# wangshiwen-ai-hku/video-styler

Measured on AMD Instinct MI355X. Metric: denoising steps/sec, Wan2.1-VACE-14B 832x480x73, higher is better.
Workload: dtype bf16; 1 GPU; Wan2.1-VACE-14B 832x480x73: 40 DiT + 8 VACE blocks, CFG 5.0 as one batch-2 forward + Euler; model=Wan2.1-VACE-14B, global_batch=1, seq_len=29640, parallelism=single, lora=merged (zero runtime cost, as the reference's GeneralLoRALoader), step_exec=hipGraph replay, sampler=flow-match Euler, cfg 5.0, shift 5.0

## Files before the change

video-styler_amd/csrc/attention_w4.hip:

```cpp
#include <cstdlib>
#include <mutex>
#include <set>
#include <type_traits>

#include "attention.h"

namespace vs_attn {
namespace {

constexpr int W4_THR = 256;
constexpr int W4_TILE = BKV * HD * 2;
constexpr int W4_SLOT = 2 * W4_TILE;
constexpr int W4_LDS = 4 * W4_SLOT;
constexpr int W4_QSLOT = W4_LDS;
constexpr int W4_LDS_BASE = W4_LDS + 16;
#ifdef VS_W4_STAMPS
__device__ unsigned long long g_w4_stamps[4][32][7];
constexpr int W4_SWN = 9;
__device__ unsigned long long g_w4_sw[4][16][W4_SWN];
constexpr int W4_STAMP_OFF = W4_LDS_BASE;
constexpr int W4_SW_OFF = W4_STAMP_OFF + 4 * 32 * 7 * 8;
constexpr int W4_LDS_ALLOC = W4_SW_OFF + 4 * 16 * W4_SWN * 8;
#else
constexpr int W4_LDS_ALLOC = W4_LDS_BASE;
#endif

struct AttnChunks {
    int nmain, npers;
    __device__ __forceinline__ void of(int x, int& cs, int& csz, int& gs) const {
        const int qx = nmain >> 3, rx = nmain & 7, qb = npers >> 3, rb = npers & 7;
        cs = x < rx ? x * (qx + 1) : rx * (qx + 1) + (x - rx) * qx;
        csz = qx + (x < rx ? 1 : 0);
        gs = qb + (x < rb ? 1 : 0);
    }
    __device__ __forceinline__ int take(unsigned* q, unsigned t0, int nxt, int lane) const {
        const int x = blockIdx.x & 7;
        int cs, csz, gs;
        of(x, cs, csz, gs);
        if (!q) return nxt + gs < cs + csz ? nxt + gs : -1;
        const unsigned t = vs_queue_value<0>(t0);
        if ((int)t < csz) return cs + (int)t;
        for (int it = 0; it < 16; ++it) {
            int vcs, vcsz, vgs;
            of((x + 1 + lane) & 7, vcs, vcsz, vgs);
            unsigned h = 0x7fffffff;
            if (lane < 7) h = __hip_atomic_load(q + ((x + 1 + lane) & 7) * VS_Q_LINE, __ATOMIC_RELAXED,
                                                __HIP_MEMORY_SCOPE_AGENT);
            const unsigned long long live = __ballot(lane < 7 && (int)h < vcsz);
            if (!live) return -1;
            const int v = (x + 1 + (int)__builtin_ctzll(live)) & 7;
            unsigned tv = 0;
            if (lane == 0) tv = vs_queue_add(q + v * VS_Q_LINE);
            tv = (unsigned)__builtin_amdgcn_readfirstlane((int)tv);
            of(v, vcs, vcsz, vgs);
            if ((int)tv < vcsz) return vcs + (int)tv;
        }
        return -1;
    }
};

template <bool REBASE>
__global__ __launch_bounds__(W4_THR, 1) void attn_fwd_w4(const AttnArgs args) {
    extern __shared__ __attribute__((aligned(16))) char smem[];
    typedef const volatile AttnArgs __attribute__((address_space(4))) ColdArgs;
    ColdArgs* cold = (ColdArgs*)__builtin_amdgcn_kernarg_segment_ptr();
    const int Sq = args.Sq, Skv_all = args.Skv, nmain = args.nmain, npers = args.npers;
    const int nsplit = args.nsplit, piece_tiles = args.piece_tiles;
    const long long ldq = args.ldq, ldk = args.ldk, ldv = args.ldv, ldo = args.ldo;
    const float c = args.c;

    int piece = -1, kv_begin = 0, Skv = Skv_all;
    int cur;
    const bool pers = (int)blockIdx.x < npers;
    const AttnChunks chunks{nmain, npers};
    const int tid = threadIdx.x, lane = tid & 63;
    if (pers) {
        int cs, csz, gs;
        chunks.of(blockIdx.x & 7, cs, csz, gs);
        cur = (int)(blockIdx.x >> 3) < csz ? cs + (int)(blockIdx.x >> 3) : -1;
    } else {
        const int t = blockIdx.x - npers;
        cur = nmain + t / nsplit;
        piece = t % nsplit;
        kv_begin = piece * piece_tiles * BKV;
        Skv = min(Skv_all - kv_begin, piece_tiles * BKV);
    }
    const int wave = __builtin_amdgcn_readfirstlane(tid >> 6);
    if (pers && args.queue) {
        volatile LDS_AS int* qs = (volatile LDS_AS int*)(uintptr_t)((unsigned)(uintptr_t)smem + W4_QSLOT);
        if (wave == 0) {
            const unsigned t0 = vs_queue_issue(args.queue + (blockIdx.x & 7) * VS_Q_LINE);
            const int id = chunks.take(args.queue, t0, -1, lane);
            if (lane == 0) *qs = id;
        }
        __syncthreads();
        cur = __builtin_amdgcn_readfirstlane(*qs);
    }
    if (cur < 0) {
        if (pers && args.queue && tid == 0) vs_queue_done(args.queue, 9, npers);
        return;
    }
    const int r = lane & 31, hh = lane >> 5;

    auto item_bh = [&](int g, int& qrow0) {
        const int nqb = cold->nqb;
        qrow0 = (g % nqb) * BQ;
        return g / nqb;
    };
    auto q_base = [&](int bh) { const int H = cold->H; return cold->Q + (long long)(bh / H) * cold->bsq + (bh % H) * HD; };
    auto k_base = [&](int bh) {
        const int H = cold->H;
        return cold->K + (long long)(bh / H) * cold->bsk + (long long)kv_begin * ldk + (bh % H) * HD;
    };
    auto v_base = [&](int bh) {
        const int H = cold->H;
        return cold->V + (long long)(bh / H) * cold->bsv + (long long)kv_begin * ldv + (bh % H) * HD;
    };
    auto o_base = [&](int bh) { const int H = cold->H; return cold->O + (long long)(bh / H) * cold->bso + (bh % H) * HD; };

    const int nkv = (Skv + BKV - 1) / BKV;
    const float npad = (float)(nkv * BKV - Skv);

    const int ldk32 = (int)ldk, ldv32 = (int)ldv;
    unsigned kvo[4], vvo[4];
#pragma unroll
    for (int i = 0; i < 4; ++i) {
        const int R = 16 * wave + 4 * i + (lane >> 4), p = lane & 15;
        kvo[i] = (unsigned)(R * ldk32 * 2 + ((p ^ (R & 15)) << 4));
        vvo[i] = (unsigned)(R * ldv32 * 2 + ((p ^ ((R & 3) << 2)) << 4));
    }
    auto rsrc4 = [&](const bf16_t* base, unsigned bytes) {
        const unsigned long long a = (unsigned long long)(uintptr_t)base;
        return i32x4_t{(int)(unsigned)a, (int)((unsigned)(a >> 32) & 0xffffu), (int)bytes, 0x00020000};
    };
    auto slab_rsrc = [&](const bf16_t* base, int ld) {
        return rsrc4(base, REBASE ? 0u : (unsigned)((Skv - 1) * ld * 2 + HD * 2));
    };
    auto dma16 = [](unsigned lds, unsigned voff, i32x4_t rs, int soff) __attribute__((always_inline)) {
        asm volatile("s_mov_b32 m0, %0\n\ts_nop 0\n\tbuffer_load_dwordx4 %1, %2, %3 offen lds"
                     :: "s"(lds), "v"(voff), "s"(rs), "s"(soff) : "m0");
    };
    int li = 0;
    int dnext = -1;
    int qrow_unused;
    const bf16_t* Kl = k_base(item_bh(cur, qrow_unused));
    const bf16_t* Vl = v_base(item_bh(cur, qrow_unused));
    i32x4_t krs = slab_rsrc(Kl, ldk32), vrs = slab_rsrc(Vl, ldv32);
    const unsigned lds0 = (unsigned)(uintptr_t)smem + wave * 16 * 256;
    struct StageCtx { unsigned kdst, vdst; i32x4_t kr, vr; int ks, vs; } sc;
    auto stage_begin = [&](int T) __attribute__((always_inline)) {
        sc.kdst = lds0 + (T & 3) * W4_SLOT;
        sc.vdst = sc.kdst + W4_TILE;
        const int kv0 = li * BKV;
        sc.kr = krs;
        sc.vr = vrs;
        sc.ks = kv0 * ldk32 * 2;
        sc.vs = kv0 * ldv32 * 2;
        if constexpr (REBASE) {
            const int rows = min(BKV, Skv - kv0);
            sc.kr = rsrc4(Kl + (long long)kv0 * ldk, (unsigned)((rows - 1) * ldk32 * 2 + HD * 2));
            sc.vr = rsrc4(Vl + (long long)kv0 * ldv, (unsigned)((rows - 1) * ldv32 * 2 + HD * 2));
            sc.ks = 0;
            sc.vs = 0;
        }
    };
    auto stage_piece = [&](int i) __attribute__((always_inline)) {
        if (i < 4)
            dma16(sc.kdst + i * 1024, kvo[i], sc.kr, sc.ks);
        else
            dma16(sc.vdst + (i - 4) * 1024, vvo[i - 4], sc.vr, sc.vs);
    };
    auto piece_go = [&](int i) __attribute__((always_inline)) {
        if (i < 4)
            asm volatile("buffer_load_dwordx4 %0, %1, %2 offen lds" :: "v"(kvo[i]), "s"(sc.kr), "s"(sc.ks) : "memory");
        else
            asm volatile("buffer_load_dwordx4 %0, %1, %2 offen lds" :: "v"(vvo[i - 4]), "s"(sc.vr), "s"(sc.vs) : "memory");
    };
    auto m0_step = [&](int i) __attribute__((always_inline)) {
        if (i == 4) asm volatile("s_add_u32 m0, m0, %0" :: "i"(W4_TILE - 3 * 1024) : "memory");
        else asm volatile("s_add_u32 m0, m0, 0x400" ::: "memory");
    };
    auto stage_next = [&]() __attribute__((always_inline)) {
        if (++li == nkv) {
            li = 0;
            if (dnext >= 0) {
                const int bh = item_bh(dnext, qrow_unused);
                Kl = k_base(bh);
                Vl = v_base(bh);
                krs = slab_rsrc(Kl, ldk32);
                vrs = slab_rsrc(Vl, ldv32);
                dnext = -1;
            }
        }
    };
    auto stage = [&](int T) __attribute__((always_inline)) {
        stage_begin(T);
#pragma unroll
        for (int i = 0; i < 8; ++i) stage_piece(i);
        stage_next();
    };

    bf16x8_t qf[2][8];
    auto load_q = [&](const bf16_t* qb0, int q0v) __attribute__((always_inline)) {
        bf16x8_t raw[2][8];
#pragma unroll
        for (int rb = 0; rb < 2; ++rb) {
            const int qrow = min(q0v + 32 * rb + r, Sq - 1);
            const bf16_t* src = qb0 + (long long)qrow * ldq + 8 * hh;
#pragma unroll
            for (int j = 0; j < 8; ++j) raw[rb][j] = *reinterpret_cast<const bf16x8_t*>(src + 16 * j);
        }
#pragma unroll
        for (int rb = 0; rb < 2; ++rb)
#pragma unroll
            for (int j = 0; j < 8; ++j) {
#pragma unroll
                for (int e = 0; e < 8; ++e) qf[rb][j][e] = (__bf16)((float)raw[rb][j][e] * c);
                asm volatile("" : "+a"(qf[rb][j]));
            }
    };

    int koff[8], voff[4];
#pragma unroll
    for (int j = 0; j < 8; ++j) {
        koff[j] = r * 256 + (((2 * j + hh) ^ (r & 15)) << 4);
        asm volatile("" : "+v"(koff[j]));
    }
    {
        const int g4 = lane >> 4, q4 = (lane & 15) >> 2, p4 = lane & 3;
#pragma unroll
        for (int dt = 0; dt < 4; ++dt) {
            voff[dt] = W4_TILE + (4 * (g4 >> 1) + q4) * 256 + ((dt ^ q4) << 6) + 32 * (g4 & 1) + 8 * p4;
            asm volatile("" : "+v"(voff[dt]));
        }
    }
    const unsigned smem_base = (unsigned)(uintptr_t)smem;
    auto lds16 = [&](unsigned addr) {
        return *reinterpret_cast<const LDS_AS bf16x8_t*>((const LDS_AS char*)(uintptr_t)addr);
    };
    auto tr8 = [&](unsigned addr) {
        return __builtin_amdgcn_ds_read_tr16_b64_v4i16((LDS_AS i16x4_t*)(uintptr_t)addr);
    };

    f32x16_t o[2][4];
#pragma unroll
    for (int rb = 0; rb < 2; ++rb)
#pragma unroll
        for (int dt = 0; dt < 4; ++dt)
#pragma unroll
            for (int i = 0; i < 16; ++i) o[rb][dt][i] = 0.f;
    float lsum[2] = {0.f, 0.f};
    auto row_sum = [&](int rb) { return lsum[rb] + __shfl_xor(lsum[rb], 32); };
    f32x16_t zero;
#pragma unroll
    for (int i = 0; i < 16; ++i) zero[i] = 0.f;


    auto finish = [&](bf16_t* ob, int qrow0, int gi) __attribute__((always_inline)) {
        float lt[2];
#pragma unroll
        for (int rb = 0; rb < 2; ++rb) lt[rb] = row_sum(rb) - npad;
        if (piece >= 0) {
            float* pp = args.part + ((long long)(gi - nmain) * nsplit + piece) * BQ * PROW + wave * 64 * PROW;
#pragma unroll
            for (int rb = 0; rb < 2; ++rb) {
                float* pr = pp + (32 * rb + r) * PROW;
#pragma unroll
                for (int dt = 0; dt < 4; ++dt)
#pragma unroll
                    for (int gi4 = 0; gi4 < 4; ++gi4)
                        *reinterpret_cast<f32x4_t*>(pr + 32 * dt + 8 * gi4 + 4 * hh) =
                            f32x4_t{o[rb][dt][4 * gi4], o[rb][dt][4 * gi4 + 1], o[rb][dt][4 * gi4 + 2],
                                    o[rb][dt][4 * gi4 + 3]};
                if (hh == 0) *reinterpret_cast<f32x2_t*>(pr + HD) = f32x2_t{0.f, lt[rb]};
            }
            return;
        }
        const bool ok = lt[0] >= W4_LMIN && lt[0] <= NC_LMAX && lt[1] >= W4_LMIN && lt[1] <= NC_LMAX;
        if (__any(!ok) && lane == 0) nc_list_item(cold->flags, cold->nc_cap, gi);
#pragma unroll
        for (int rb = 0; rb < 2; ++rb) {
            const float inv = 1.f / lt[rb];
            const int row = qrow0 + 32 * rb + r;
            bf16_t* op = ob + (long long)row * ldo + 8 * hh;
#pragma unroll
            for (int dt = 0; dt < 4; ++dt)
#pragma unroll
                for (int gp = 0; gp < 2; ++gp) {
                    const int gi = 2 * gp;
                    const unsigned ax = pack2(o[rb][dt][4 * gi] * inv, o[rb][dt][4 * gi + 1] * inv);
                    const unsigned ay = pack2(o[rb][dt][4 * gi + 2] * inv, o[rb][dt][4 * gi + 3] * inv);
                    const unsigned bx = pack2(o[rb][dt][4 * gi + 4] * inv, o[rb][dt][4 * gi + 5] * inv);
                    const unsigned by = pack2(o[rb][dt][4 * gi + 6] * inv, o[rb][dt][4 * gi + 7] * inv);
                    const auto sx = __builtin_amdgcn_permlane32_swap(ax, bx, false, false);
                    const auto sy = __builtin_amdgcn_permlane32_swap(ay, by, false, false);
                    if (row < Sq)
                        *reinterpret_cast<u32x4_t*>(op + 16 * (2 * dt + gp)) = u32x4_t{sx[0], sy[0], sx[1], sy[1]};
                }
        }
    };

    bf16x8_t kf0[8], kf1[8], vfa[8], vfb[8];
    f32x16_t s0[2], s1a[2], s1b[2];
    u32x4_t p0a[2][2], p0b[2][2], p1[2][2];
    auto fence = [] { __builtin_amdgcn_sched_barrier(0); };
#ifdef VS_W4_STAMPS
    unsigned long long stv[7] = {0, 0, 0, 0, 0, 0, 0};
    int st_it = -1;
    auto stamp = [&](int k) __attribute__((always_inline)) {
        if (st_it >= 0) asm volatile("s_memtime %0" : "=s"(stv[k]));
    };
    auto stamp_store = [&](int st, int lo, int hi) __attribute__((always_inline)) {
        if (st >= 0 && lane == 0)
            for (int k = lo; k < hi; ++k)
                *reinterpret_cast<volatile LDS_AS unsigned long long*>(
                    (LDS_AS char*)(uintptr_t)(smem_base + W4_STAMP_OFF + 8 * ((wave * 32 + st) * 7 + k))) = stv[k];
    };
    unsigned long long swv[W4_SWN] = {};
    int sw_i = 0;
    auto swst = [&](int k) __attribute__((always_inline)) {
        if (blockIdx.x == 0 && sw_i < 16) asm volatile("s_memtime %0\n\ts_waitcnt lgkmcnt(0)" : "=s"(swv[k]) :: "memory");
    };
    auto sw_store = [&]() __attribute__((always_inline)) {
        if (blockIdx.x == 0 && sw_i < 16) {
            asm volatile("s_waitcnt lgkmcnt(0)" ::: "memory");
            if (lane == 0)
                for (int k = 0; k < W4_SWN; ++k)
                    *reinterpret_cast<volatile LDS_AS unsigned long long*>(
                        (LDS_AS char*)(uintptr_t)(smem_base + W4_SW_OFF + 8 * ((wave * 16 + sw_i) * W4_SWN + k))) = swv[k];
        }
        ++sw_i;
    };
#else
    auto stamp = [](int) {};
    auto swst = [](int) {};
    auto sw_store = [] {};
#endif
    unsigned kbs[8], vbs[4];
    auto kbase = [&](int T) __attribute__((always_inline)) {
#pragma unroll
        for (int j = 0; j < 8; ++j) {
            kbs[j] = smem_base + (T & 3) * W4_SLOT + koff[j];
            asm volatile("" : "+v"(kbs[j]));
        }
    };
    auto vbase = [&](int T) __attribute__((always_inline)) {
#pragma unroll
        for (int dt = 0; dt < 4; ++dt) vbs[dt] = smem_base + (T & 3) * W4_SLOT + voff[dt];
    };
    auto rdK = [&](bf16x8_t& d, int kb, int j) __attribute__((always_inline)) {
        d = lds16(kbs[j] + kb * 32 * 256);
    };
    auto rdV = [&](bf16x8_t& d, int ks, int dt) __attribute__((always_inline)) {
        const unsigned a0 = vbs[dt] + ks * 16 * 256;
        const i16x4_t v0 = tr8(a0), v1 = tr8(a0 + 8 * 256);
        d = __builtin_shufflevector(__builtin_bit_cast(bf16x4_t, v0), __builtin_bit_cast(bf16x4_t, v1), 0, 1, 2,
                                    3, 4, 5, 6, 7);
    };
    auto mfV = [&](const bf16x8_t& vf, const u32x4_t (&pkv)[2][2], int ksl, int dt) __attribute__((always_inline)) {
#pragma unroll
        for (int rb = 0; rb < 2; ++rb)
        {
            o[rb][dt] = __builtin_amdgcn_mfma_f32_32x32x16_bf16(vf, __builtin_bit_cast(bf16x8_t, pkv[rb][ksl]),
                                                                 o[rb][dt], 0, 0, 0);
            asm volatile("" : "+a"(o[rb][dt]));
        }
    };
    auto mfV1 = [&](const bf16x8_t& vf, const u32x4_t (&pkv)[2][2], int ksl, int dt, int rb) __attribute__((always_inline)) {
        o[rb][dt] = __builtin_amdgcn_mfma_f32_32x32x16_bf16(vf, __builtin_bit_cast(bf16x8_t, pkv[rb][ksl]), o[rb][dt], 0, 0, 0);
        asm volatile("" : "+a"(o[rb][dt]));
    };
    auto smp = [&](const f32x16_t& sv, int e, u32x4_t (&pkd)[2], int rb) __attribute__((always_inline)) {
        const float pa = __builtin_amdgcn_exp2f(sv[e]), pb = __builtin_amdgcn_exp2f(sv[e + 1]);
        lsum[rb] += pa + pb;
        const bf16x2_t w = {(__bf16)pa, (__bf16)pb};
        unsigned wu = __builtin_bit_cast(unsigned, w);
        asm volatile("" : "+v"(lsum[rb]), "+v"(wu));
        pkd[e >> 3][(e >> 1) & 3] = wu;
    };
    auto smp_e = [&](const f32x16_t& sv, int e, float& pa, float& pb) __attribute__((always_inline)) {
        pa = __builtin_amdgcn_exp2f(sv[e]);
        pb = __builtin_amdgcn_exp2f(sv[e + 1]);
        asm volatile("" : "+v"(pa), "+v"(pb));
    };
    auto smp_f = [&](float pa, float pb, int e, u32x4_t (&pkd)[2], int rb) __attribute__((always_inline)) {
        lsum[rb] += pa + pb;
        const bf16x2_t w = {(__bf16)pa, (__bf16)pb};
        unsigned wu = __builtin_bit_cast(unsigned, w);
        asm volatile("" : "+v"(lsum[rb]), "+v"(wu));
        pkd[e >> 3][(e >> 1) & 3] = wu;
    };
    auto mfK1 = [&](const bf16x8_t& kf, int j, f32x16_t (&sv)[2], int rb) __attribute__((always_inline)) {
        if (j == 0)
            asm volatile("v_mfma_f32_32x32x16_bf16 %0, %1, %2, 0" : "=v"(sv[rb]) : "v"(kf), "a"(qf[rb][j]));
        else
            asm volatile("v_mfma_f32_32x32x16_bf16 %0, %1, %2, %0" : "+v"(sv[rb]) : "v"(kf), "a"(qf[rb][j]));
    };
    auto sync = [&](int T, auto first_c) __attribute__((always_inline)) {
        fence();
        stamp(3);
        if constexpr (!decltype(first_c)::value)
            asm volatile("s_mov_b32 m0, %0" :: "s"(lds0 + ((T + 3) & 3) * W4_SLOT) : "m0");
        asm volatile("s_waitcnt lgkmcnt(0)\n\ts_waitcnt vmcnt(8)\n\ts_barrier" ::: "memory");
        fence();
        stamp(4);
#ifdef VS_W4_STAMPS
        stamp_store(st_it, 0, 4);
#endif
        stage_begin(T + 3);
    };
    int nxt = -1, qv = 0;
    auto iteration = [&](int T, f32x16_t (&s1c)[2], const f32x16_t (&s1p)[2], u32x4_t (&p0c)[2][2],
                         const u32x4_t (&p0p)[2][2], auto first_c) __attribute__((always_inline)) {
        constexpr bool FIRST = decltype(first_c)::value;
#ifdef VS_W4_STAMPS
        if (st_it >= 0) {
            asm volatile("s_waitcnt lgkmcnt(0)" ::: "memory");
            stamp_store(st_it, 4, 7);
        }
        st_it = (blockIdx.x == 0 && !FIRST && T >= 8 && T < 40) ? T - 8 : -1;
#endif
        stamp(0);
#pragma unroll
        for (int j = 0; j < 8; ++j) {
            float pa = 0.f, pb = 0.f;
            rdK(kf1[j], 1, j);
            mfK1(kf0[j], j, s0, 0);
            fence();
            if (!FIRST) smp_e(s1p[0], 2 * j, pa, pb);
            fence();
            mfK1(kf0[j], j, s0, 1);
            fence();
            if (!FIRST) smp_f(pa, pb, 2 * j, p1[0], 0);
            fence();
        }
        stamp(1);
        if (!FIRST) vbase(T - 1);
#pragma unroll
        for (int j = 0; j < 8; ++j) {
            float pa = 0.f, pb = 0.f;
            if (!FIRST) rdV(vfa[j], j >> 2, j & 3);
            mfK1(kf1[j], j, s1c, 0);
            fence();
            if (!FIRST) smp_e(s1p[1], 2 * j, pa, pb);
            fence();
            mfK1(kf1[j], j, s1c, 1);
            fence();
            if (!FIRST) smp_f(pa, pb, 2 * j, p1[1], 1);
            fence();
        }
        stamp(2);
#pragma unroll
        for (int i = 0; i < 8; ++i) {
            if (!FIRST) {
                if (i < 4) {
                    rdV(vfb[2 * i], 2 + (i >> 1), (2 * i) & 3);
                    rdV(vfb[2 * i + 1], 2 + (i >> 1), (2 * i + 1) & 3);
                }
                mfV(vfa[i], p0p, i >> 2, i & 3);
            }
            smp(s0[0], 2 * i, p0c[0], 0);
            smp(s0[1], 2 * i, p0c[1], 1);
            fence();
        }
        sync(T, first_c);
        kbase(T + 1);
#pragma unroll
        for (int i = 0; i < 8; ++i) {
            if (FIRST) stage_piece(i);
            else piece_go(i);
            if (FIRST && i == 0)
                qv = *(volatile LDS_AS int*)(uintptr_t)(smem_base + W4_QSLOT);
            rdK(kf0[i], 0, i);
            if (!FIRST) {
                mfV1(vfb[i], p1, i >> 2, i & 3, 0);
                fence();
                if (i < 7) m0_step(i + 1);
                fence();
                mfV1(vfb[i], p1, i >> 2, i & 3, 1);
            }
            fence();
#ifdef VS_W4_STAMPS
            if (i == 3) stamp(6);
#endif
        }
        stamp(5);
        if constexpr (FIRST) {
            nxt = __builtin_amdgcn_readfirstlane(qv);
            dnext = nxt;
        }
        stage_next();
    };
    auto drain = [&](int TL, const f32x16_t (&s1l)[2], const u32x4_t (&p0l)[2][2]) __attribute__((always_inline)) {
        vbase(TL);
#pragma unroll
        for (int j = 0; j < 8; ++j) {
            rdV(vfa[j], j >> 2, j & 3);
            smp(s1l[0], 2 * j, p1[0], 0);
            fence();
        }
#pragma unroll
        for (int j = 0; j < 8; ++j) {
            rdV(vfb[j], 2 + (j >> 2), j & 3);
            smp(s1l[1], 2 * j, p1[1], 1);
            fence();
        }
#pragma unroll
        for (int i = 0; i < 8; ++i) mfV(vfa[i], p0l, i >> 2, i & 3);
#pragma unroll
        for (int i = 0; i < 8; ++i) mfV(vfb[i], p1, i >> 2, i & 3);
    };
    stage(0);
    stage(1);
    fence();
    asm volatile("s_waitcnt vmcnt(8)\n\ts_barrier" ::: "memory");
    fence();
    stage(2);
    kbase(0);
#pragma unroll
    for (int i = 0; i < 8; ++i) rdK(kf0[i], 0, i);
    int T = 0, q0 = 0;
    int bh = item_bh(cur, q0);
    q0 += 64 * wave;
    unsigned* const qw = pers ? args.queue : nullptr;
    auto next_q = [&](int after) __attribute__((always_inline)) {
        unsigned t0 = 0;
#ifdef VS_W4_STAMPS
        swst(6);
        asm volatile("s_waitcnt vmcnt(0)" ::: "memory");
        swst(7);
#endif
        if (qw && wave == 0) t0 = vs_queue_issue(qw + (blockIdx.x & 7) * VS_Q_LINE);
        load_q(q_base(bh), q0);
#ifdef VS_W4_STAMPS
        swst(8);
#endif
        if (wave == 0) {
            const int id = pers ? chunks.take(qw, t0, after, lane) : -1;
            if (lane == 0) *(volatile LDS_AS int*)(uintptr_t)(smem_base + W4_QSLOT) = id;
        }
    };
    next_q(cur);
    for (;;) {
#pragma unroll
        for (int rb = 0; rb < 2; ++rb) {
            lsum[rb] = 0.f;
#pragma unroll
            for (int dt = 0; dt < 4; ++dt)
#pragma unroll
                for (int i = 0; i < 16; ++i) o[rb][dt][i] = 0.f;
        }
        swst(0);
        iteration(T, s1a, s1b, p0a, p0b, std::true_type{});
        swst(1);
        ++T;
        int t = 1;
        for (; t + 1 < nkv; t += 2) {
            iteration(T, s1b, s1a, p0b, p0a, std::false_type{});
            ++T;
            iteration(T, s1a, s1b, p0a, p0b, std::false_type{});
            ++T;
        }
        swst(2);
        const int bh_done = bh, q0_done = q0;
        if (nxt >= 0) {
            bh = item_bh(nxt, q0);
            q0 += 64 * wave;
        }
        if (t < nkv) {
            iteration(T, s1b, s1a, p0b, p0a, std::false_type{});
            ++T;
            swst(3);
            drain(T - 1, s1b, p0b);
        } else {
            swst(3);
            drain(T - 1, s1a, p0a);
        }
        swst(4);
        finish(o_base(bh_done), q0_done, cur);
        if (nxt >= 0) next_q(nxt);
        swst(5);
        sw_store();
        if (nxt < 0) break;
        cur = nxt;
    }
    asm volatile("s_waitcnt vmcnt(0)" ::: "memory");
    if (qw && tid == 0) vs_queue_done(qw, 9, npers);
#ifdef VS_W4_STAMPS
    asm volatile("s_waitcnt lgkmcnt(0)" ::: "memory");
    stamp_store(st_it, 4, 7);
    __syncthreads();
    if (blockIdx.x == 0)
        for (int i = lane; i < 32 * 7; i += 64)
            (&g_w4_stamps[wave][0][0])[i] = *reinterpret_cast<volatile unsigned long long*>(smem + W4_STAMP_OFF + 8 * (wave * 32 * 7 + i));
    if (blockIdx.x == 0)
        for (int i = lane; i < 16 * W4_SWN; i += 64)
            (&g_w4_sw[wave][0][0])[i] = *reinterpret_cast<volatile unsigned long long*>(smem + W4_SW_OFF + 8 * (wave * 16 * W4_SWN + i));
#endif
}

}

hipError_t attn_w4_launch(const AttnArgs& args, bool rebase, unsigned grid, hipStream_t stream) {
    void (*kern)(AttnArgs) = rebase ? attn_fwd_w4<true> : attn_fwd_w4<false>;
    static std::mutex mu;
    static std::set<const void*> done;
    {
        std::lock_guard<std::mutex> lock(mu);
        if (done.insert((const void*)kern).second)
            (void)hipFuncSetAttribute((const void*)kern, hipFuncAttributeMaxDynamicSharedMemorySize, W4_LDS_ALLOC);
    }
    hipLaunchKernelGGL(kern, dim3(grid), dim3(W4_THR), W4_LDS_ALLOC, stream, args);
    return hipGetLastError();
}

}

#ifdef VS_W4_STAMPS
extern "C" int vs_debug_w4_switch(unsigned long long* host_out) {
    return hipMemcpyFromSymbol(host_out, HIP_SYMBOL(vs_attn::g_w4_sw), sizeof(vs_attn::g_w4_sw)) == hipSuccess ? 0 : 2;
}
extern "C" int vs_debug_w4_stamps(unsigned long long* host_out) {
    return hipMemcpyFromSymbol(host_out, HIP_SYMBOL(vs_attn::g_w4_stamps), sizeof(vs_attn::g_w4_stamps)) == hipSuccess ? 0 : 2;
}
#endif
```

Measured before the change: 0.4040 steps/s.

## Prefetch next Q tile into LDS via async DMA during attention KV loop

The persistent attention kernel now stages most of the next work item's Q rows into a per-wave LDS area with buffer DMA loads, issued early in the current item's KV loop. The remaining Q fragments and the work-queue ticket load are issued before the drain and finish steps, so their latency overlaps epilogue work instead of stalling afterwards. The loop is also reshaped so the iteration parity always ends on the same buffer, which removes the branch on the tail. The change needs up to 28 KB of extra LDS, which may reduce occupancy, and adds more complex vmcnt accounting.

```diff
diff --git a/video-styler_amd/csrc/attention_w4.hip b/video-styler_amd/csrc/attention_w4.hip
--- a/video-styler_amd/csrc/attention_w4.hip
+++ b/video-styler_amd/csrc/attention_w4.hip
@@ -13,7 +13,13 @@
 constexpr int W4_SLOT = 2 * W4_TILE;
 constexpr int W4_LDS = 4 * W4_SLOT;
 constexpr int W4_QSLOT = W4_LDS;
-constexpr int W4_LDS_BASE = W4_LDS + 16;
+#ifdef VS_W4_STAMPS
+constexpr int W4_NQL = 4;
+#else
+constexpr int W4_NQL = 7;
+#endif
+constexpr int W4_QST_OFF = W4_LDS + 16;
+constexpr int W4_LDS_BASE = W4_QST_OFF + 4 * W4_NQL * 1024;
 #ifdef VS_W4_STAMPS
 __device__ unsigned long long g_w4_stamps[4][32][7];
 constexpr int W4_SWN = 9;
@@ -24,6 +30,7 @@
 #else
 constexpr int W4_LDS_ALLOC = W4_LDS_BASE;
 #endif
+static_assert(W4_LDS_ALLOC <= 160 * 1024, "attn_fwd_w4: LDS of one CU");
 
 struct AttnChunks {
     int nmain, npers;
@@ -33,12 +40,11 @@
         csz = qx + (x < rx ? 1 : 0);
         gs = qb + (x < rb ? 1 : 0);
     }
-    __device__ __forceinline__ int take(unsigned* q, unsigned t0, int nxt, int lane) const {
+    __device__ __forceinline__ int take(unsigned* q, unsigned t, int nxt, int lane) const {
         const int x = blockIdx.x & 7;
         int cs, csz, gs;
         of(x, cs, csz, gs);
         if (!q) return nxt + gs < cs + csz ? nxt + gs : -1;
-        const unsigned t = vs_queue_value<0>(t0);
         if ((int)t < csz) return cs + (int)t;
         for (int it = 0; it < 16; ++it) {
             int vcs, vcsz, vgs;
@@ -90,7 +96,7 @@
         volatile LDS_AS int* qs = (volatile LDS_AS int*)(uintptr_t)((unsigned)(uintptr_t)smem + W4_QSLOT);
         if (wave == 0) {
             const unsigned t0 = vs_queue_issue(args.queue + (blockIdx.x & 7) * VS_Q_LINE);
-            const int id = chunks.take(args.queue, t0, -1, lane);
+            const int id = chunks.take(args.queue, vs_queue_value<0>(t0), -1, lane);
             if (lane == 0) *qs = id;
         }
         __syncthreads();
@@ -201,21 +207,41 @@
     };
 
     bf16x8_t qf[2][8];
-    auto load_q = [&](const bf16_t* qb0, int q0v) __attribute__((always_inline)) {
-        bf16x8_t raw[2][8];
+    const unsigned qst0 = (unsigned)(uintptr_t)smem + W4_QST_OFF + wave * W4_NQL * 1024;
+    auto stage_q = [&](const bf16_t* qb0, int q0v) __attribute__((always_inline)) {
+        const i32x4_t rs = rsrc4(qb0, (unsigned)((unsigned long long)(Sq - 1) * ldq * 2 + HD * 2));
+#pragma unroll
+        for (int p = 0; p < W4_NQL; ++p) {
+            const int qrow = min(q0v + 32 * (p >> 3) + r, Sq - 1);
+            const unsigned vo = (unsigned)((unsigned long long)qrow * ldq * 2) + 16 * hh;
+            dma16(qst0 + p * 1024, vo, rs, 32 * (p & 7));
+        }
+    };
+    bf16x8_t qraw[2][8];
+    auto q_issue = [&](const bf16_t* qb0, int q0v, auto staged_c) __attribute__((always_inline)) {
+        constexpr int NS = decltype(staged_c)::value ? W4_NQL : 0;
 #pragma unroll
         for (int rb = 0; rb < 2; ++rb) {
             const int qrow = min(q0v + 32 * rb + r, Sq - 1);
             const bf16_t* src = qb0 + (long long)qrow * ldq + 8 * hh;
 #pragma unroll
-            for (int j = 0; j < 8; ++j) raw[rb][j] = *reinterpret_cast<const bf16x8_t*>(src + 16 * j);
-        }
+            for (int j = 0; j < 8; ++j)
+                if (8 * rb + j >= NS) qraw[rb][j] = *reinterpret_cast<const bf16x8_t*>(src + 16 * j);
+        }
+    };
+    auto q_finish = [&](auto staged_c) __attribute__((always_inline)) {
+        constexpr int NS = decltype(staged_c)::value ? W4_NQL : 0;
+        if (NS && nkv < 3) asm volatile("s_waitcnt vmcnt(0)" ::: "memory");
+#pragma unroll
+        for (int p = 0; p < NS; ++p)
+            qraw[p >> 3][p & 7] = *reinterpret_cast<const LDS_AS bf16x8_t*>(
+                (const LDS_AS char*)(uintptr_t)(qst0 + p * 1024 + lane * 16));
 #pragma unroll
         for (int rb = 0; rb < 2; ++rb)
 #pragma unroll
             for (int j = 0; j < 8; ++j) {
 #pragma unroll
-                for (int e = 0; e < 8; ++e) qf[rb][j][e] = (__bf16)((float)raw[rb][j][e] * c);
+                for (int e = 0; e < 8; ++e) qf[rb][j][e] = (__bf16)((float)qraw[rb][j][e] * c);
                 asm volatile("" : "+a"(qf[rb][j]));
             }
     };
@@ -520,27 +546,35 @@
 #pragma unroll
     for (int i = 0; i < 8; ++i) rdK(kf0[i], 0, i);
     int T = 0, q0 = 0;
-    int bh = item_bh(cur, q0);
+    const bf16_t *qb, *qb_n = nullptr;
+    bf16_t *ob, *ob_n = nullptr;
+    int q0_n = 0;
+    {
+        const int bh = item_bh(cur, q0);
+        qb = q_base(bh);
+        ob = o_base(bh);
+    }
     q0 += 64 * wave;
     unsigned* const qw = pers ? args.queue : nullptr;
-    auto next_q = [&](int after) __attribute__((always_inline)) {
-        unsigned t0 = 0;
-#ifdef VS_W4_STAMPS
+    unsigned tq0 = 0;
+    auto next_q_issue = [&](auto staged_c) __attribute__((always_inline)) {
+        tq0 = 0;
+        if (qw && wave == 0) tq0 = vs_queue_issue(qw + (blockIdx.x & 7) * VS_Q_LINE);
+        q_issue(qb, q0, staged_c);
         swst(6);
-        asm volatile("s_waitcnt vmcnt(0)" ::: "memory");
+    };
+    auto next_q_finish = [&](int after, auto staged_c) __attribute__((always_inline)) {
         swst(7);
-#endif
-        if (qw && wave == 0) t0 = vs_queue_issue(qw + (blockIdx.x & 7) * VS_Q_LINE);
-        load_q(q_base(bh), q0);
-#ifdef VS_W4_STAMPS
+        q_finish(staged_c);
         swst(8);
-#endif
+        const unsigned tq = vs_queue_value<16 - (decltype(staged_c)::value ? W4_NQL : 0)>(tq0);
         if (wave == 0) {
-            const int id = pers ? chunks.take(qw, t0, after, lane) : -1;
+            const int id = pers ? chunks.take(qw, tq, after, lane) : -1;
             if (lane == 0) *(volatile LDS_AS int*)(uintptr_t)(smem_base + W4_QSLOT) = id;
         }
     };
-    next_q(cur);
+    next_q_issue(std::false_type{});
+    next_q_finish(cur, std::false_type{});
     for (;;) {
 #pragma unroll
         for (int rb = 0; rb < 2; ++rb) {
@@ -551,34 +585,50 @@
                 for (int i = 0; i < 16; ++i) o[rb][dt][i] = 0.f;
         }
         swst(0);
-        iteration(T, s1a, s1b, p0a, p0b, std::true_type{});
-        swst(1);
-        ++T;
+        auto prefetch_next = [&]() __attribute__((always_inline)) {
+            if (nxt >= 0) {
+                const int bh_n = item_bh(nxt, q0_n);
+                q0_n += 64 * wave;
+                qb_n = q_base(bh_n);
+                ob_n = o_base(bh_n);
+                stage_q(qb_n, q0_n);
+            }
+        };
         int t = 1;
-        for (; t + 1 < nkv; t += 2) {
+        if (nkv & 1) {
+            iteration(T, s1a, s1b, p0a, p0b, std::true_type{});
+            swst(1);
+            ++T;
+            prefetch_next();
+        } else {
+            iteration(T, s1b, s1a, p0b, p0a, std::true_type{});
+            swst(1);
+            ++T;
+            prefetch_next();
+            iteration(T, s1a, s1b, p0a, p0b, std::false_type{});
+            ++T;
+            ++t;
+        }
+        for (; t < nkv; t += 2) {
             iteration(T, s1b, s1a, p0b, p0a, std::false_type{});
             ++T;
             iteration(T, s1a, s1b, p0a, p0b, std::false_type{});
             ++T;
         }
         swst(2);
-        const int bh_done = bh, q0_done = q0;
+        bf16_t* const ob_done = ob;
+        const int q0_done = q0;
         if (nxt >= 0) {
-            bh = item_bh(nxt, q0);
-            q0 += 64 * wave;
-        }
-        if (t < nkv) {
-            iteration(T, s1b, s1a, p0b, p0a, std::false_type{});
-            ++T;
-            swst(3);
-            drain(T - 1, s1b, p0b);
-        } else {
-            swst(3);
-            drain(T - 1, s1a, p0a);
-        }
+            qb = qb_n;
+            ob = ob_n;
+            q0 = q0_n;
+        }
+        swst(3);
+        if (nxt >= 0) next_q_issue(std::true_type{});
+        drain(T - 1, s1a, p0a);
         swst(4);
-        finish(o_base(bh_done), q0_done, cur);
-        if (nxt >= 0) next_q(nxt);
+        finish(ob_done, q0_done, cur);
+        if (nxt >= 0) next_q_finish(nxt, std::true_type{});
         swst(5);
         sw_store();
         if (nxt < 0) break;
```

New measurement: 0.4045 steps/s, median of 6. Within noise of the previous version (+0.1%).
